# Labbeti/conette-audio-captioning

Hardware: AMD Instinct MI355X
Metric: clips_per_sec (higher is better)
Workload: dtype bf16; 1 GPU; B=64/GPU x 10 s @ 32 kHz clips, ConvNeXt encoder + beam-3 KV-cached decode (min 3 / max 20 tokens, V=5631), synthetic seeded checkpoint; batch_per_gpu=64, global_batch=64, beam_size=3, parallelism=dp1, world_size_observed=1, allreduce_of_ones=1, decode_group=2, decode_streams=2, encode_streams=1, input_batches_rotated=4

## Files before the change

### conette-audio-captioning_amd/build.py

```python
from __future__ import annotations

import json
import os
import shutil
import subprocess
import sys
from concurrent.futures import ThreadPoolExecutor

HERE = os.path.dirname(os.path.abspath(__file__))
CSRC = os.path.join(HERE, "csrc")
LIB = os.path.join(HERE, "libconette_hip.so")
SOURCES = ["api.hip", "frontend.hip", "encoder.hip", "decoder.hip"]
FLAGS = ["--offload-arch=gfx950", "-O3", "-std=c++17", "-fPIC", "-Wno-unused-value"]
if os.environ.get("CN_G2_PROF"):
    FLAGS.append("-DCN_G2_PROF")
for knob in ("FE_NOFILL", "FE_POISON", "FE_NW", "FE_VARIANT"):
    if os.environ.get(knob):
        FLAGS.append(f"-D{knob}" + ("" if os.environ[knob] == "1" and knob != "FE_NW" else "=" + os.environ[knob]))
if os.environ.get("CN_EXTRA_FLAGS"):
    FLAGS += os.environ["CN_EXTRA_FLAGS"].split()
if os.environ.get("CN_DB_ROWS"):
    FLAGS.append("-DDB_ROWS=" + os.environ["CN_DB_ROWS"])
if os.environ.get("CN_DB_ROWS_SP"):
    FLAGS.append("-DDB_ROWS_SP=" + os.environ["CN_DB_ROWS_SP"])
if os.environ.get("CN_DB_WIDE_ROWS"):
    FLAGS.append("-DDB_WIDE_ROWS=" + os.environ["CN_DB_WIDE_ROWS"])
if os.environ.get("CN_DB_WIDE_ROWS_SP"):
    FLAGS.append("-DDB_WIDE_ROWS_SP=" + os.environ["CN_DB_WIDE_ROWS_SP"])
if os.environ.get("CN_DB_WIDE_R"):
    FLAGS.append("-DDB_WIDE_R=" + os.environ["CN_DB_WIDE_R"])
for _k in ("CN_DW96_S", "CN_DW96_TH", "CN_DW192_S", "CN_DW192_TH"):
    if os.environ.get(_k):
        FLAGS.append(f"-D{_k}=" + os.environ[_k])
if os.environ.get("CN_FW_SPLIT"):
    FLAGS.append("-DCN_FW_SPLIT=" + os.environ["CN_FW_SPLIT"])
if os.environ.get("CN_FW_TH"):
    FLAGS.append("-DCN_FW_TH=" + os.environ["CN_FW_TH"])


def hipcc() -> str:
    for cand in (shutil.which("hipcc"), "/opt/rocm/bin/hipcc"):
        if cand and os.path.exists(cand):
            return cand
    raise RuntimeError("hipcc not found")


FILE_FLAGS = {} if os.environ.get("CN_ALLOW_PK_HAZARD") else {"frontend.hip": ["-fno-slp-vectorize"], "decoder.hip": ["-fno-slp-vectorize"]}


SIDECAR = os.path.join(HERE, "libconette_hip.build.json")
# ... 121 lines not shown
```

### conette-audio-captioning_amd/csrc/api.hip

```cpp
#include <math.h>
#include <stdarg.h>
#include <stdlib.h>

#include <string>
#include <unordered_map>
#include <vector>

#include "ctx.h"
#include <algorithm>
#include "mlp_rc2.h"
#include "mlp_rs16.h"
#include "mlp_sp.h"
#include "down_fused.h"

static thread_local char g_err[512] = "";

void cn_set_error(const char* fmt, ...) {
  va_list ap;
  va_start(ap, fmt);
  vsnprintf(g_err, sizeof(g_err), fmt, ap);
  va_end(ap);
}

extern "C" const char* conette_last_error(void) { return g_err; }
// ... 227 lines not shown
  }
  conette_ctx* ctx = new conette_ctx();
  memset(ctx, 0, sizeof(*ctx));
  ctx->cfg = *cfg;
  ctx->rt = new CnRuntime();
  ctx->esize = (cfg->precision == CONETTE_PREC_BF16 || cfg->precision == CONETTE_PREC_F16) ? 2 : 4;
  ctx->f16 = cfg->precision == CONETTE_PREC_F16 ? 1 : 0;
  ctx->sp16 = cfg->precision == CONETTE_PREC_F16X2 ? 1 : 0;
  {
    int dev = 0, n_cu = 0;
    if (hipGetDevice(&dev) != hipSuccess || hipDeviceGetAttribute(&n_cu, hipDeviceAttributeMultiprocessorCount, dev) != hipSuccess ||
        n_cu <= 0)
      n_cu = 256;
    ctx->n_cu = n_cu;
  }
  size_t total = (1 << 20) + (size_t)CN_N_BINS * CN_N_MELS * 4;
  for (int i = 0; i < n_tensors; ++i) total += cn_align((size_t)numel[i] * 4) + 256;
  if (cfg->precision == CONETTE_PREC_F16X2) {
    total += 8u << 20;
    total += (size_t)cfg->n_layers * ((size_t)12 * 131072 + (size_t)(cfg->d_ff / 256 + 1) * 4 * 131072 + 4096);
  }
  ctx->arena_bytes = total;
  hipError_t e = hipMalloc((void**)&ctx->arena, total);
  if (e != hipSuccess) {
    cn_set_error("create: hipMalloc(%zu) -> %s", total, hipGetErrorString(e));
    delete ctx->rt;
    delete ctx;
    return CN_ERR_HIP;
  }
  Builder B;
// ... 424 lines not shown
```

### conette-audio-captioning_amd/csrc/ctx.h

```cpp
#pragma once
#include "../../include/conette_hip.h"
#include "common.h"

#define CN_N_MELS 224
#define CN_N_FFT 1024
#define CN_HOP 320
#define CN_N_BINS 513
#define CN_N_TAGS 527
#define CN_FEAT 768
#define CN_MAX_LAYERS 12

static const int CN_DEPTHS[4] = {3, 3, 9, 3};
static const int CN_DIMS[4] = {96, 192, 384, 768};

struct CnBlockW {
  const float* dw_w;
  const unsigned* dw_wp;
  const float* dw_b;
  const float* ln_w;
  const float* ln_b;
  const void* w1;
  const float* b1;
  const void* w2;
  const float* b2;
// ... 59 lines not shown
  const float* norm_b;
  const void* head_w;
  const float* head_b;
  const void* proj_w;
  const float* proj_b;
  const void* kv_w;
  const float* kv_b;
  CnLayerW layers[CN_MAX_LAYERS];
  const float* emb;
  const float* pe;
  int pe_len;
  const void* cls_w;
  const float* cls_b;
  int n_cu;
  int enc_reserved_cus;
  int forcing_stepwise;
  int score_vsplit;
  char* arena;
  size_t arena_bytes;
  size_t arena_used;
};

void cn_prof_begin(conette_ctx* ctx, int cls, hipStream_t s);
void cn_prof_end(conette_ctx* ctx, int cls, hipStream_t s);
struct CnProfScope {
  conette_ctx* ctx;
  int cls;
  hipStream_t s;
  CnProfScope(conette_ctx* c, int k, hipStream_t st) : ctx(c), cls(k), s(st) {
    if (ctx->prof_mask & (1u << cls)) cn_prof_begin(ctx, cls, s);
// ... 23 lines not shown
```

### conette-audio-captioning_amd/csrc/decoder.hip

```cpp
#include "ctx.h"
#include <stdlib.h>

#include <type_traits>

#include "gemm2.h"
#include "dec_ffn.h"
#include "dec_score.h"

#define CN_MAX_BEAM 16
#define CN_MAX_PRED 64
#define FF2_SPLITS 8
static int ff2_splits_default() { return 4; }

template <typename T>
__global__ void cn_cvt_kernel(const float* __restrict__ in, T* __restrict__ out, size_t n) {
  for (size_t i = (size_t)blockIdx.x * blockDim.x + threadIdx.x; i < n; i += (size_t)gridDim.x * blockDim.x)
    out[i] = cn_from_f32<T>(in[i]);
}

__global__ void cn_init_state_kernel(int B, int beam, int maxp, const int* __restrict__ bos, int* n_active, int* slot,
                                     float* sum_lp, int* prefix, int* anc, int* cur_tok, int* out_preds,
                                     float* out_avg, int* out_len, int* sizes, int pad_id, int* trace_sel,
                                     float* trace_val, int* live, float* margins) {
  const int R = B * beam;
// ... 1180 lines not shown
    if (value < 0) {
      cn_set_error("set_option: score vocabulary split %d < 0", value);
      return CN_ERR_ARG;
    }
    ctx->score_vsplit = value;
    return CN_OK;
  }
  if (option == CONETTE_OPT_ENCODE_RESERVED_CUS) {
    if (value < 0 || value > ctx->n_cu / 2) {
      cn_set_error("set_option: reserved CUs %d outside 0 .. %d", value, ctx->n_cu / 2);
      return CN_ERR_ARG;
    }
    ctx->enc_reserved_cus = value;
    return CN_OK;
  }
  cn_set_error("set_option: unknown option %d", option);
  return CN_ERR_ARG;
}

template <typename... A>
static int dec_check_model(const conette_ctx* ctx, const char* who, int len, int min_pred, const char* len_fmt, A... len_args) {
  if (len < 1 || len > CN_MAX_PRED || len > ctx->pe_len || min_pred < 0) {
    cn_set_error(len_fmt, len_args...);
    return CN_ERR_ARG;
  }
  if (ctx->cfg.d_model != 256 || ctx->cfg.nhead != 8) {
    cn_set_error("%s: kernels are specialised for d_model=256, nhead=8", who);
    return CN_ERR_ARG;
  }
  return CN_OK;
// ... 387 lines not shown
```

### conette-audio-captioning_amd/csrc/down_fused.h

```cpp
#pragma once
__device__ void cn_watch_stat(float v);
#include "mlp_rc2.h"

template <int CP> struct DownGeom {
  static constexpr int K = 4 * CP, N = 2 * CP, KS = K / 16, NT = N / 32, CH = CP / 16;
  static constexpr size_t STREAM_BYTES = (size_t)KS * NT * 1024;
  static constexpr size_t TOTAL_BYTES = STREAM_BYTES + N * 4;
};

template <typename HT>
static __global__ void pk_down_fused(const float* __restrict__ src, const float* __restrict__ g, const float* __restrict__ b,
                                     const float* __restrict__ bias, int N, int C, HT* __restrict__ dst) {
  const int K = 4 * C, KS = K / 16, NT = N / 32;
  const int u = blockIdx.x * blockDim.x + threadIdx.x;
  if (u < N) {
    float a = bias[u];
    for (int k = 0; k < K; ++k) a = fmaf(src[((size_t)u * C + k % C) * 4 + k / C], b[k % C], a);
    ((float*)((char*)dst + (size_t)KS * NT * 1024))[u] = a;
  }
  if (u >= KS * NT * 64) return;
  const int l = u & 63, t = (u >> 6) % NT, s = (u >> 6) / NT;
  const int n = 32 * t + cn_rc2_chan(l & 31);
#pragma unroll
  for (int i = 0; i < 8; ++i) {
// ... 106 lines not shown
    constexpr int s = Q / G::NT, t = Q % G::NT;
    acc[t] = cn_mma32(f[Q % R], a[s], acc[t]);
    __builtin_amdgcn_sched_barrier(0);
    if constexpr (Q + 1 < NM) step<Q + 1>(wl, a, acc, f);
  }
  template <int Q>
  static __device__ __forceinline__ void run(const char* wl, const cn_h8<HT> (&a)[G::KS], f32x16 (&acc)[G::NT]) {
    cn_h8<HT> f[R];
#pragma unroll
    for (int q = 0; q < PRE; ++q) f[q] = *(const cn_h8<HT>*)(wl + q * 1024);
    __builtin_amdgcn_sched_barrier(0);
    step<0>(wl, a, acc, f);
  }
};

template <int CP, int NW, typename HT, typename XT>
__global__ __launch_bounds__(NW * 64) void cn_down_fused_kernel(const XT* __restrict__ X, int H, int W, long P,
                                                                const HT* __restrict__ WS, XT* __restrict__ OUT) {
  typedef DownGeom<CP> G;
  constexpr int KS = G::KS, NT = G::NT, CH = G::CH, N = G::N;
  extern __shared__ __attribute__((aligned(16))) char smem[];
  const int tid = threadIdx.x, lane = tid & 63;
  const int wave = __builtin_amdgcn_readfirstlane(tid >> 6);
  constexpr int PIECES = (int)(G::STREAM_BYTES / 1024);
  for (int i = wave; i < PIECES; i += NW)
    __builtin_amdgcn_global_load_lds((const __attribute__((address_space(1))) void*)((const char*)WS + (size_t)i * 1024 + lane * 16),
                                     (__attribute__((address_space(3))) void*)(smem + i * 1024), 16, 0, 0);
  const float* biasp = (const float*)((const char*)WS + G::STREAM_BYTES);
  const long n_tiles = (P + 31) >> 5;
  const long t_lo = (long)blockIdx.x * n_tiles / gridDim.x, t_hi = (long)(blockIdx.x + 1) * n_tiles / gridDim.x;
  asm volatile("s_waitcnt vmcnt(0)" ::: "memory");
  __syncthreads();
  const char* wl = smem + lane * 16;
  for (long tile = t_lo + wave; tile < t_hi; tile += NW) {
    cn_h8<HT> a[KS];
    cn_down_operand<CP, 0, 4, HT, XT>(X, H, W, P, tile, lane, a);
    f32x16 acc[NT];
#pragma unroll
    for (int t = 0; t < NT; ++t)
#pragma unroll
      for (int i = 0; i < 16; ++i) acc[t][i] = 0.f;
    DownMma<CP, HT>::template run<0>(wl, a, acc);
    cn_down_store<CP, XT>(OUT, biasp, P, tile, lane, acc);
  }
}

template <int CP, int NW, typename HT, typename XT>
static int cn_launch_down_fused(const XT* X, int B, int H, int W, const void* WS, XT* OUT, int n_blocks, hipStream_t s) {
  typedef DownGeom<CP> G;
  constexpr int SMEM = (int)G::STREAM_BYTES;
  static_assert(SMEM <= 160 * 1024, "the packed weights must fit in LDS");
  const long P = (long)B * (H / 2) * (W / 2);
  CN_TRY(cn_configure_lds((const void*)cn_down_fused_kernel<CP, NW, HT, XT>, SMEM));
  const int grid = cn_rc2_grid((int)((P + 31) / 32), NW, n_blocks);
  hipLaunchKernelGGL((cn_down_fused_kernel<CP, NW, HT, XT>), dim3((unsigned)grid), dim3(NW * 64), SMEM, s, X, H, W, P, (const HT*)WS, OUT);
  CN_LAUNCH_CHECK();
  return CN_OK;
}

template <int CP, int NW, int KSTEP, int NST, typename HT> struct DownRing {
  typedef DownGeom<CP> G;
  static constexpr int NT = G::NT, KS = G::KS, NSTEP = KS / KSTEP, FR = KSTEP * NT, SB = FR * 1024;
  static constexpr int DPW = FR / NW, PRE = 6, R = PRE + 1;
  static_assert(KS % KSTEP == 0 && NSTEP % NST == 0 && FR % NW == 0, "ring geometry");
  static constexpr int SMEM = NST * SB;

  static __device__ __forceinline__ void stage(const char* wsrc, char* smem, int wave, int g) {
    const char* src = wsrc + (size_t)(g % NSTEP) * SB;
    char* dst = smem + (g % NST) * SB;
#pragma unroll
// ... 82 lines not shown
```

### conette-audio-captioning_amd/csrc/encoder.hip

```cpp
#include <stddef.h>

#include "ctx.h"
#include <type_traits>

__device__ int g_cn_nonfinite;
__device__ __forceinline__ void cn_watch_stat(float v) {
  if (!(__builtin_fabsf(v) <= 3.0e38f)) atomicAdd(&g_cn_nonfinite, 1);
}

#include "gemm2.h"
#include "mlp_rc2.h"
#include "mlp_rs16.h"
#include "mlp_sp.h"
#include "down_fused.h"

template <typename XT>
__global__ __launch_bounds__(256) void cn_stem_mfma_kernel(const float* __restrict__ in, int F, int H0, long n_pos,
                                                           const float* __restrict__ w , const float* __restrict__ bias,
                                                           const float* __restrict__ ln_w, const float* __restrict__ ln_b,
                                                           XT* __restrict__ out) {
  __shared__ __attribute__((aligned(16))) float s_p[3 * 96];
  for (int i = threadIdx.x; i < 3 * 96; i += 256) s_p[i] = i < 96 ? bias[i] : i < 192 ? ln_w[i - 96] : ln_b[i - 192];
  const int lane = threadIdx.x & 63, j = lane & 31, h = lane >> 5;
  float a[3][8];
#pragma unroll
  for (int t = 0; t < 3; ++t)
#pragma unroll
    for (int s = 0; s < 8; ++s) a[t][s] = w[(4 * (s >> 1) + 2 * h + (s & 1)) * 96 + 32 * t + cn_rc2_chan(j)];
  __syncthreads();
  const long n_tiles = (n_pos + 31) >> 5;
  const long n_waves = (long)gridDim.x * 4;
  for (long tile = (long)blockIdx.x * 4 + (threadIdx.x >> 6); tile < n_tiles; tile += n_waves) {
    const long pos = tile * 32 + j;
    const long p = pos < n_pos ? pos : n_pos - 1;
    const int wq = (int)(p % 56);
// ... 732 lines not shown
    g.W[i] = g.W[i - 1] / 2;
  }
  return g;
}

extern "C" int32_t conette_num_frames(int32_t n_samples) { return n_samples / CN_HOP + 1; }
extern "C" int32_t conette_num_audio_frames(int32_t n_samples) { return enc_geom(n_samples).H[3]; }

struct EncWs {
  float* logmel;
  void* x;
  void* y;
  void* h;
  void* fe_t;
  void* clip_t;
  size_t total;
};
static EncWs enc_ws(const conette_ctx* ctx, int B, int L, char* base) {
  const EncGeom g = enc_geom(L);
  const size_t es = ctx->esize;
  const size_t n0 = (size_t)B * g.H[0] * g.W[0] * 96;
  EncWs w;
  size_t off = 0;
  auto take = [&](size_t bytes) {
    char* p = base ? base + off : nullptr;
    off += cn_align(bytes);
    return p;
  };
  w.logmel = (float*)take((size_t)B * g.F * CN_N_MELS * 4);
  w.x = take((n0 + 32 * 96) * 4);
  w.y = take((n0 + 32 * 96) * es);
  w.h = take(n0 * 4 * es);
  w.fe_t = take((size_t)B * g.H[3] * CN_FEAT * es);
  w.clip_t = take((size_t)B * CN_FEAT * es);
  w.total = off;
  return w;
}

extern "C" size_t conette_encode_workspace_bytes(const conette_ctx* ctx, int32_t batch, int32_t n_samples) {
  return enc_ws(ctx, batch, n_samples, nullptr).total;
}

template <typename T, typename XT>
static int dwconv_dispatch(int C, const XT* x, int B, int H, int W, const CnBlockW& bw, T* y, hipStream_t s) {
  switch (C) {
    case 96: return launch_dwconv<T, XT, 96, CN_DW96_S, sizeof(XT) == 2 ? CN_DW96_TH : 8>(x, B, H, W, bw, y, s);
    case 192: return launch_dwconv<T, XT, 192, CN_DW192_S, sizeof(XT) == 2 ? CN_DW192_TH : 8>(x, B, H, W, bw, y, s);
    case 384:
      if (W == 14) return launch_dwconv_fw<T, XT, 384, 14, CN_FW_TH, CN_FW_SPLIT>(x, B, H, bw, y, s);
// ... 17 lines not shown
  if (dst) {
    hipLaunchKernelGGL(cn_tap_widen_kernel, dim3((unsigned)((n + 255) / 256 < 4096 ? (n + 255) / 256 : 4096)), dim3(256), 0, s, src, dst, n);
    CN_LAUNCH_CHECK();
  }
  return CN_OK;
}

template <typename T, typename XT>
static int encode_impl(conette_ctx* ctx, const float* wave, int B, int L, float* frame_embs, float* clip_probs,
                       const conette_encode_taps* taps, char* wsp, hipStream_t s) {
  const EncGeom g = enc_geom(L);
  EncWs ws = enc_ws(ctx, B, L, wsp);
  T* y = (T*)ws.y;
  T* hbuf = (T*)ws.h;
  XT* const wsx = (XT*)ws.x;
  {
    CnProfScope ps(ctx, CONETTE_PROF_FRONTEND, s);
    CN_TRY(cn_frontend(ctx, wave, B, L, ws.logmel, s));
  }
  if (taps) CN_TRY(tap_copy(taps->logmel, ws.logmel, (size_t)B * g.F * CN_N_MELS, s));
  {
    const long n_pos = (long)B * g.H[0] * g.W[0];
    CnProfScope ps(ctx, CONETTE_PROF_STEM, s);
    const long n_tiles = (n_pos + 31) / 32;
    const unsigned grid = (unsigned)std::min<long>((n_tiles + 3) / 4, 8L * ctx->n_cu);
    hipLaunchKernelGGL((cn_stem_mfma_kernel<XT>), dim3(grid), dim3(256), 0, s, ws.logmel, g.F, g.H[0], n_pos, ctx->stem_w, ctx->stem_b,
                       ctx->stem_ln_w, ctx->stem_ln_b, wsx);
    CN_LAUNCH_CHECK();
    if (taps) CN_TRY(tap_copy(taps->stem, wsx, (size_t)n_pos * 96, s));
  }
  XT* xc = wsx;
  int blk = 0;
  for (int st = 0; st < 4; ++st) {
    const int C = CN_DIMS[st], H = g.H[st], W = g.W[st];
    const long P = (long)B * H * W;
    if (st > 0) {
      const int Cp = CN_DIMS[st - 1], Hp = g.H[st - 1], Wp = g.W[st - 1];
      const long n_in = (long)B * Hp * Wp;
      const CnDownW& dw = ctx->down[st - 1];
      CnProfScope ps(ctx, CONETTE_PROF_DOWNSAMPLE, s);
      bool fused_down = false;
      if constexpr (CnIsH16<T>::value) if (Cp <= 192 && dw.fused != nullptr) {
        XT* xo = xc == wsx ? (XT*)ws.h : wsx;
        const int nb = ctx->n_cu - ctx->enc_reserved_cus;
        if (Cp == 96) CN_TRY((cn_launch_down_fused<96, 8, T, XT>(xc, B, Hp, Wp, dw.fused, xo, nb, s)));
        else CN_TRY((cn_launch_down_fused_ring<192, 4, 4, 3, T, XT>(xc, B, Hp, Wp, dw.fused, xo, nb, s)));
        xc = xo;
        if (taps) CN_TRY(tap_copy(taps->down[st], xc, (size_t)P * C, s));
        fused_down = true;
      }
      if (!fused_down) {
      const int ppb = Cp == 96 ? 32 : 16;
      const dim3 pg((unsigned)((n_in + ppb - 1) / ppb));
      if (Cp == 96)
        hipLaunchKernelGGL((cn_ln_patchify_kernel<T, XT, 96>), pg, dim3(256), 0, s, xc, Hp, Wp, n_in, dw.ln_w, dw.ln_b, y);
      else if (Cp == 192)
        hipLaunchKernelGGL((cn_ln_patchify_kernel<T, XT, 192>), pg, dim3(256), 0, s, xc, Hp, Wp, n_in, dw.ln_w, dw.ln_b, y);
      else
        hipLaunchKernelGGL((cn_ln_patchify_kernel<T, XT, 384>), pg, dim3(256), 0, s, xc, Hp, Wp, n_in, dw.ln_w, dw.ln_b, y);
      CN_LAUNCH_CHECK();
// ... 1 lines not shown
      CN_TRY(cn_mm(y, 4 * Cp, (const T*)dw.w, 4 * Cp, (int)P, C, 4 * Cp, epi, s));
      xc = wsx;
      if (taps) CN_TRY(tap_copy(taps->down[st], xc, (size_t)P * C, s));
      }
    }
    for (int b = 0; b < CN_DEPTHS[st]; ++b, ++blk) {
      const CnBlockW& bw = ctx->blocks[blk];
      {
        CnProfScope ps(ctx, CONETTE_PROF_DWCONV_LN, s);
        CN_TRY((dwconv_dispatch<T, XT>(C, xc, B, H, W, bw, y, s)));
      }
      bool fused = false;
      if constexpr (std::is_same<T, sp16_t>::value) {
        if (bw.mlp_sp != nullptr && C <= 192) {
          CnProfScope ps(ctx, CONETTE_PROF_PW1_GEMM, s);
          const int nb = ctx->n_cu - ctx->enc_reserved_cus;
          if (C == 96) CN_TRY((cn_launch_mlp_sp_ring<96, CN_SP_NW96, CN_SP_NST96>(y, bw.mlp_sp, xc, (int)P, nb, s)));
          else CN_TRY((cn_launch_mlp_sp_ring<192, 8, 3>(y, bw.mlp_sp, xc, (int)P, nb, s)));
          fused = true;
        }
      }
      if constexpr (CnIsH16<T>::value) if (!fused) {
        if (bw.mlp_stream != nullptr && C <= 384) {
          CnProfScope ps(ctx, CONETTE_PROF_PW1_GEMM, s);
          const T* wsm = (const T*)bw.mlp_stream;
          if (C == 96) CN_TRY((cn_launch_mlp_rc2_resident<96, 12, 1>(y, wsm, xc, (int)P, ctx->n_cu - ctx->enc_reserved_cus, s)));
          else if (C == 192) CN_TRY((cn_launch_mlp_rc2_ring<192, 8, CN_RC2_NCK(192), CN_RC2_NCK(192) == 2 ? 3 : 5>(y, wsm, xc, (int)P, ctx->n_cu - ctx->enc_reserved_cus, s)));
          else CN_TRY((cn_launch_mlp_rs16<384, 4, 3, 8>(y, wsm, xc, (int)P, ctx->n_cu - ctx->enc_reserved_cus, s)));
          fused = true;
        }
      }
      if (!fused) {
        {
          CnProfScope ps(ctx, CONETTE_PROF_PW1_GEMM, s);
          constexpr int kAct = CnGeluAct<T>::value;
          EpiBiasAct<T, kAct> e1{bw.b1, hbuf, 4 * C, kAct};
          CN_TRY(cn_mm(y, C, (const T*)bw.w1, C, (int)P, 4 * C, C, e1, s));
        }
        {
          CnProfScope ps(ctx, CONETTE_PROF_PW2_GEMM, s);
          EpiResidT<XT> e2{bw.b2, bw.scale, xc, xc, C};
          CN_TRY(cn_mm(hbuf, 4 * C, (const T*)bw.w2, 4 * C, (int)P, C, 4 * C, e2, s));
        }
// ... 92 lines not shown
```

### conette-audio-captioning_amd/csrc/mlp_rc2.h

```cpp
#pragma once
#include "common.h"

template <int C, int NCK> struct Rc2Geom {
  static constexpr int KS1 = C / 16, NT2 = C / 32, NCH = C / 8;
  static constexpr int F1 = KS1 + 1, F2 = 2 * NT2;
  static constexpr int NSTEP = NCH / NCK;
  static constexpr int FRAGS = NCK * (F1 + F2);
  static constexpr int STEP_BYTES = FRAGS * 1024;
  static constexpr size_t STREAM_BYTES = (size_t)NSTEP * STEP_BYTES;
  static constexpr size_t TOTAL_BYTES = STREAM_BYTES + NT2 * 1024;
};
__host__ __device__ constexpr int cn_rc2_chan(int m) { return (m & 19) | ((m & 4) << 1) | ((m & 8) >> 1); }

#define CN_MLP_XSCALE 0.5f
template <typename HT> __device__ __forceinline__ float cn_gelu_mlp(float x) {
  return cn_gelu_e1_half<__is_same(HT, half_t) ? 5 : 3>(x);
}

template <typename HT>
static __global__ void pk_mlp_rc2(const float* __restrict__ W1, const float* __restrict__ b1, const float* __restrict__ W2,
                           const float* __restrict__ b2, const float* __restrict__ scale, int C, int NCK,
                           HT* __restrict__ dst) {
  const int KS1 = C / 16, NT2 = C / 32, NCH = C / 8, F1 = KS1 + 1, F2 = 2 * NT2, FRAGS = NCK * (F1 + F2), NSTEP = NCH / NCK;
  const int u = blockIdx.x * blockDim.x + threadIdx.x;
// ... 201 lines not shown
      if ((r & 3) + 8 * (r >> 2) < plim) {
#pragma unroll
        for (int t = 0; t < NT2; ++t) row[voff + 32 * t] = O[t][r] + bb[t];
      }
    }
  }
};

static inline int cn_rc2_grid(int n_tiles, int waves_per_block, int max_blocks) {
  const int block_tiles = cn_cdiv(n_tiles, waves_per_block);
  if (max_blocks < 1) max_blocks = 1;
  const int rounds = cn_cdiv(block_tiles, max_blocks);
  return cn_cdiv(block_tiles, rounds);
}

template <int C, int NW, int NCK, typename HT = bf16_t, int ABL = 0, typename XT = float>
__global__ __launch_bounds__(NW * 64) void cn_mlp_rc2_resident_kernel(const HT* __restrict__ Y, const HT* __restrict__ WS,
                                                                      XT* __restrict__ X, int M) {
  typedef Rc2Geom<C, NCK> G;
  typedef Rc2Wave<C, NCK, HT, XT> W;
  typedef cn_h8<HT> hx8;
  extern __shared__ __attribute__((aligned(16))) char smem[];
  const int tid = threadIdx.x, lane = tid & 63;
  const int wave = __builtin_amdgcn_readfirstlane(tid >> 6);
  constexpr int TOTAL = G::NSTEP * G::FRAGS;
  for (int i = wave; i < TOTAL; i += NW)
    __builtin_amdgcn_global_load_lds((const __attribute__((address_space(1))) void*)((const char*)WS + (size_t)i * 1024 + lane * 16),
                                     (__attribute__((address_space(3))) void*)(smem + i * 1024), 16, 0, 0);
  const char* bbf = (const char*)WS + G::STREAM_BYTES + lane * 16;
  const int n_tiles = (M + 31) >> 5;
  const int t_lo = (int)((long)blockIdx.x * n_tiles / gridDim.x), t_hi = (int)((long)(blockIdx.x + 1) * n_tiles / gridDim.x);
  hx8 ones;
#pragma unroll
  for (int i = 0; i < 8; ++i) ones[i] = (HT)((lane < 32 && i < 2) ? 1.0f : 0.0f);
  hx8 fy[G::KS1];
  int tile = t_lo + wave;
  if (tile < t_hi) W::load_y(Y, tile * 32, lane, fy);
  asm volatile("s_waitcnt vmcnt(0)" ::: "memory");
  __syncthreads();
  const char* wl = smem + lane * 16;
  for (; tile < t_hi; tile += NW) {
    f32x16 O[G::NT2];
    if constexpr (ABL & 1) {
#pragma unroll
      for (int t = 0; t < G::NT2; ++t) O[t] = W::zero16();
    } else {
      W::init_o(X, bbf, ones, tile * 32, lane, O);
    }
#pragma unroll 1
    for (int j = 0; j < G::NSTEP; ++j) W::step(wl + j * G::STEP_BYTES, fy, ones, O);
    if constexpr (!(ABL & 8))
      if (tile + NW < t_hi) W::load_y(Y, (tile + NW) * 32, lane, fy);
    if constexpr (ABL & 2) {
      if (O[0][0] == 12345.678f) W::store_o(X, tile * 32, M, lane, O);
    } else {
      W::store_o(X, tile * 32, M, lane, O);
    }
  }
}

template <int C, int NW, int NCK, int ABL = 0, typename HT, typename XT>
static int cn_launch_mlp_rc2_resident(const HT* Y, const HT* WS, XT* X, int M, int n_blocks, hipStream_t s) {
  constexpr int SMEM = (int)Rc2Geom<C, NCK>::STREAM_BYTES;
  static_assert(SMEM <= 160 * 1024, "resident variant: the weight stream must fit in LDS");
  CN_TRY(cn_configure_lds((const void*)cn_mlp_rc2_resident_kernel<C, NW, NCK, HT, ABL, XT>, SMEM));
  const int grid = cn_rc2_grid((M + 31) / 32, NW, n_blocks);
  hipLaunchKernelGGL((cn_mlp_rc2_resident_kernel<C, NW, NCK, HT, ABL, XT>), dim3((unsigned)grid), dim3(NW * 64), SMEM, s, Y, WS, X, M);
  CN_LAUNCH_CHECK();
  return CN_OK;
}

template <int C, int NW, int NCK, int NST, int PROF = 0, typename HT = bf16_t, typename XT = float>
__global__ __launch_bounds__(NW * 64) void cn_mlp_rc2_ring_kernel(const HT* __restrict__ Y, const HT* __restrict__ WS,
                                                                  XT* __restrict__ X, int M, unsigned long long* prof = nullptr) {
  unsigned long long tacc[5] = {0, 0, 0, 0, 0}, tprev = 0, nstep = 0;
  auto stamp = [&](int i) {
    if constexpr (PROF) {
      const unsigned long long t = clock64();
      tacc[i] += t - tprev;
      tprev = t;
    }
  };
  if constexpr (PROF) tprev = clock64();
  typedef Rc2Geom<C, NCK> G;
  typedef Rc2Wave<C, NCK, HT, XT> W;
  typedef cn_h8<HT> hx8;
  constexpr int FR = G::FRAGS, SB = G::STEP_BYTES;
  constexpr int DPW_LO = FR / NW, N_HI = FR % NW;
  extern __shared__ __attribute__((aligned(16))) char smem[];
  const int tid = threadIdx.x, lane = tid & 63;
  const int wave = __builtin_amdgcn_readfirstlane(tid >> 6);
  const char* bbf = (const char*)WS + G::STREAM_BYTES + lane * 16;

  const int n_tiles = (M + 31) >> 5;
  const int t_lo = (int)((long)blockIdx.x * n_tiles / gridDim.x), t_hi = (int)((long)(blockIdx.x + 1) * n_tiles / gridDim.x);
  const int max_it = (t_hi - t_lo + NW - 1) / NW;

  const unsigned voff = lane * 16;
  const unsigned lds0 = cn_lds_addr(smem);
  auto stage = [&](int g) {
    const char* src = (const char*)WS + (size_t)(g % G::NSTEP) * SB;
    const unsigned dst = lds0 + (unsigned)((g % NST) * SB);
#pragma unroll
    for (int i = 0; i < DPW_LO + 1; ++i) {
      const int piece = wave + i * NW;
      if (i < DPW_LO || wave < N_HI) cn_dma16_s(src + piece * 1024, voff, dst + piece * 1024);
    }
  };
  hx8 ones;
#pragma unroll
  for (int i = 0; i < 8; ++i) ones[i] = (HT)((lane < 32 && i < 2) ? 1.0f : 0.0f);

#pragma unroll
  for (int g = 0; g < NST - 1; ++g) stage(g);
  hx8 fy[G::KS1];
  if (t_lo + wave < t_hi) W::load_y(Y, (t_lo + wave) * 32, lane, fy);
  const char* wl = smem + lane * 16;
  int g = 0;
  for (int it = 0; it < max_it; ++it) {
    const int tile = t_lo + wave + it * NW;
    const bool valid = tile < t_hi;
    f32x16 O[G::NT2];
    if (valid) W::init_o(X, bbf, ones, tile * 32, lane, O);
    {
      __builtin_amdgcn_s_waitcnt(0x0F70);
    }
    for (int j = 0; j < G::NSTEP; ++j, ++g) {
      stamp(4);
      if (N_HI > 0 && wave < N_HI) asm volatile("s_waitcnt vmcnt(%0)" ::"n"((NST - 2) * (DPW_LO + 1)) : "memory");
      else asm volatile("s_waitcnt vmcnt(%0)" ::"n"((NST - 2) * DPW_LO) : "memory");
      stamp(0);
      __builtin_amdgcn_s_barrier();
      stamp(1);
      stage(g + NST - 1);
      stamp(2);
      if (valid) W::step(wl + (g % NST) * SB, fy, ones, O);
      stamp(3);
      if constexpr (PROF) nstep += valid;
    }
    if (tile + NW < t_hi) W::load_y(Y, (tile + NW) * 32, lane, fy);
    if (valid) W::store_o(X, tile * 32, M, lane, O);
  }
  asm volatile("s_waitcnt vmcnt(0)" ::: "memory");
  if constexpr (PROF) {
    if (lane == 0 && prof) {
#pragma unroll
      for (int i = 0; i < 5; ++i) atomicAdd(prof + i, tacc[i]);
      atomicAdd(prof + 5, nstep);
    }
  }
}

template <int C, int NW, int NCK, int NST, int PROF = 0, typename HT, typename XT>
static int cn_launch_mlp_rc2_ring(const HT* Y, const HT* WS, XT* X, int M, int n_blocks, hipStream_t s,
                                  unsigned long long* prof = nullptr) {
  constexpr int SMEM = NST * Rc2Geom<C, NCK>::STEP_BYTES;
  static_assert(SMEM <= 160 * 1024, "ring must fit in LDS");
  CN_TRY(cn_configure_lds((const void*)cn_mlp_rc2_ring_kernel<C, NW, NCK, NST, PROF, HT, XT>, SMEM));
  const int grid = cn_rc2_grid((M + 31) / 32, NW, n_blocks);
  hipLaunchKernelGGL((cn_mlp_rc2_ring_kernel<C, NW, NCK, NST, PROF, HT, XT>), dim3((unsigned)grid), dim3(NW * 64), SMEM, s, Y, WS, X, M, prof);
  CN_LAUNCH_CHECK();
  return CN_OK;
}
```

### conette-audio-captioning_amd/engine.py

```python
from __future__ import annotations

import ctypes as C
import os
from typing import Any, Dict, Optional, Tuple

import torch

_HERE = os.path.dirname(os.path.abspath(__file__))
LIB_PATH = os.path.join(_HERE, "libconette_hip.so")

PREC_F32 = 0
PREC_BF16 = 1
PREC_F16X2 = 2
PREC_F16 = 4
N_MELS = 224
FEAT = 768
N_TAGS = 527

EXPORTS = (
    "conette_last_error", "conette_abi_version", "conette_create", "conette_destroy", "conette_num_frames",
    "conette_num_audio_frames", "conette_encode_workspace_bytes", "conette_decode_workspace_bytes",
    "conette_frontend_logmel", "conette_encode", "conette_decode", "conette_resample", "conette_resample_len",
    "conette_set_option", "conette_profile_enable", "conette_profile_read", "conette_stream_create_masked",
    "conette_stream_destroy", "conette_forcing_workspace_bytes", "conette_forcing",
# ... 4 lines not shown
    "mixed16": {"greedy": (0.032, 0.0, 0.0), "beam": (0.045, 0.0, 0.005), "wide": (0.08, 0.0, 0.005)},
    "f16": {"greedy": (0.063, 0.0, 0.0), "beam": (0.082, 0.0, 0.008), "wide": (0.13, 0.0, 0.008)},
    "bf16+f16dec": {"greedy": (0.20, 0.0, 0.0), "beam": (0.37, 0.0, 0.026), "wide": (0.65, 0.0, 0.05)},
    "bf16": {"greedy": (0.39, 0.0, 0.0), "beam": (0.58, 0.0, 0.05), "wide": (1.0, 0.0, 0.08)},
}


def cert_kind(beam: int) -> str:
    return "greedy" if int(beam) == 1 else ("beam" if int(beam) <= 5 else "wide")


CERT_DEFAULT_BASE = "mixed16"
OPT_DECODE_GRAPH = 1
OPT_DECODE_FUSION = 2
OPT_ENCODE_RESERVED_CUS = 3
OPT_FORCING_STEPWISE = 4
OPT_SCORE_VSPLIT = 5
MAX_DECODE_GRAPHS = 64
PROF_CLASSES = ("frontend", "stem", "dwconv_ln", "pw1_gemm", "pw2_gemm", "downsample", "heads", "dec_prepare",
                "dec_gemm", "dec_attn", "dec_misc", "search")


class ConetteConfigC(C.Structure):
    _fields_ = [(n, C.c_int32) for n in ("precision", "vocab_size", "d_model", "nhead", "n_layers", "d_ff", "pad_id",
                                         "bos_id", "eos_id")] + [("reserved", C.c_int32 * 7)]


class EncodeTapsC(C.Structure):
    _fields_ = [("struct_bytes", C.c_size_t), ("logmel", C.c_void_p), ("stem", C.c_void_p), ("stage_block0", C.c_void_p * 4),
                ("stage", C.c_void_p * 4), ("down", C.c_void_p * 4), ("block", C.c_void_p * 18)]
# ... 539 lines not shown
                            exact: bool = False) -> torch.Tensor:
        return self._decode_buffers(b, t, int(beam), int(max_pred), False, False, slot, margins, exact)["fe"]

    def set_decode_graph(self, enabled: bool) -> None:
        _check(self.lib.conette_set_option(self._ctx_dec, OPT_DECODE_GRAPH, int(bool(enabled))), "set_option")

    def set_decode_fusion(self, enabled: bool) -> None:
        _check(self.lib.conette_set_option(self._ctx_dec, OPT_DECODE_FUSION, int(bool(enabled))), "set_option")

    def set_forcing_stepwise(self, enabled: bool) -> None:
        _check(self.lib.conette_set_option(self._ctx_dec, OPT_FORCING_STEPWISE, int(bool(enabled))), "set_option")

    def set_encode_reserved_cus(self, n: int) -> None:
        _check(self.lib.conette_set_option(self._ctx, OPT_ENCODE_RESERVED_CUS, int(n)), "set_option")

    def decode_graph_nodes(self) -> int:
        return int(self.lib.conette_decode_graph_nodes(self._ctx_dec))

    _DEC_CLASSES = ("dec_prepare", "dec_gemm", "dec_attn", "dec_misc", "search")

    def profile_enable(self, classes=()) -> None:
        mask_enc = mask_dec = 0
        for c in classes:
            bit = 1 << PROF_CLASSES.index(c)
            if c in self._DEC_CLASSES:
                mask_dec |= bit
            else:
                mask_enc |= bit
        if self._ctx_dec is self._ctx:
            _check(self.lib.conette_profile_enable(self._ctx, mask_enc | mask_dec), "profile_enable")
# ... 24 lines not shown
```

### include/conette_hip.h

```cpp
#ifndef CONETTE_HIP_H
#define CONETTE_HIP_H

#include <stddef.h>
#include <stdint.h>

#ifdef __cplusplus
extern "C" {
#endif

#define CONETTE_ABI_VERSION 3

#define CONETTE_PREC_F32 0
#define CONETTE_PREC_BF16 1
#define CONETTE_PREC_F16X2 2


#define CONETTE_PREC_F16 4

typedef struct conette_ctx conette_ctx;

typedef struct conette_config {
  int32_t precision;
  int32_t vocab_size;
  int32_t d_model;
// ... 72 lines not shown
                   float* sum_lprobs, int32_t* lens, int32_t* out_sizes, float* tok_lprobs, float* step_logits,
                   void* workspace, size_t workspace_bytes, void* stream);

int conette_resample(const float* in, int32_t rows, int32_t n_in, int32_t orig_sr, int32_t new_sr, float* out,
                     void* stream);
int32_t conette_resample_len(int32_t n_in, int32_t orig_sr, int32_t new_sr);

int conette_stream_create_masked(const uint32_t* mask_words, int32_t n_words, void** out_stream);
int conette_stream_destroy(void* stream);

#define CONETTE_OPT_DECODE_GRAPH 1
#define CONETTE_OPT_DECODE_FUSION 2
#define CONETTE_OPT_ENCODE_RESERVED_CUS 3
#define CONETTE_OPT_FORCING_STEPWISE 4
#define CONETTE_OPT_SCORE_VSPLIT 5
int conette_set_option(conette_ctx* ctx, int32_t option, int32_t value);

int32_t conette_decode_graph_nodes(const conette_ctx* ctx);
#define CONETTE_MAX_DECODE_GRAPHS 64

#define CONETTE_PROF_FRONTEND 0
#define CONETTE_PROF_STEM 1
#define CONETTE_PROF_DWCONV_LN 2
#define CONETTE_PROF_PW1_GEMM 3
#define CONETTE_PROF_PW2_GEMM 4
#define CONETTE_PROF_DOWNSAMPLE 5
#define CONETTE_PROF_HEADS 6
#define CONETTE_PROF_DEC_PREPARE 7
#define CONETTE_PROF_DEC_GEMM 8
#define CONETTE_PROF_DEC_ATTN 9
// ... 11 lines not shown
```

Measured before the change: 13370 clips/s.

## Add atomic work-claiming tile scheduler for encoder MLP and downsample kernels

Adds a dynamic tile-claiming mode to the ConvNeXt encoder's rc2 MLP kernels and fused downsample kernel. Each wave pulls its next tile from a global atomic counter instead of a static contiguous range, which is meant to even out load imbalance and tail effects when encoder kernels share CUs with concurrent decode streams. The counters are zeroed by the stem kernel, and per-wave slots are spaced to avoid contention. The default enables it for the 96-channel MLP and downsample only. It adds atomic traffic and one readfirstlane per tile, and the ring variant gains extra LDS for the shared draw queue.

```diff
diff --git a/conette-audio-captioning_amd/build.py b/conette-audio-captioning_amd/build.py
--- a/conette-audio-captioning_amd/build.py
+++ b/conette-audio-captioning_amd/build.py
@@ -34,6 +34,8 @@
         FLAGS.append(f"-D{_k}=" + os.environ[_k])
 if os.environ.get("CN_FW_SPLIT"):
     FLAGS.append("-DCN_FW_SPLIT=" + os.environ["CN_FW_SPLIT"])
+if os.environ.get("CN_ENC_CLAIM"):
+    FLAGS.append("-DCONETTE_CLAIM_DEFAULT=" + os.environ["CN_ENC_CLAIM"])
 if os.environ.get("CN_FW_TH"):
     FLAGS.append("-DCN_FW_TH=" + os.environ["CN_FW_TH"])
 
diff --git a/conette-audio-captioning_amd/csrc/api.hip b/conette-audio-captioning_amd/csrc/api.hip
--- a/conette-audio-captioning_amd/csrc/api.hip
+++ b/conette-audio-captioning_amd/csrc/api.hip
@@ -265,6 +265,7 @@
       n_cu = 256;
     ctx->n_cu = n_cu;
   }
+  ctx->enc_claim = CONETTE_CLAIM_DEFAULT;
   size_t total = (1 << 20) + (size_t)CN_N_BINS * CN_N_MELS * 4;
   for (int i = 0; i < n_tensors; ++i) total += cn_align((size_t)numel[i] * 4) + 256;
   if (cfg->precision == CONETTE_PREC_F16X2) {
diff --git a/conette-audio-captioning_amd/csrc/ctx.h b/conette-audio-captioning_amd/csrc/ctx.h
--- a/conette-audio-captioning_amd/csrc/ctx.h
+++ b/conette-audio-captioning_amd/csrc/ctx.h
@@ -97,6 +97,8 @@
   const float* cls_b;
   int n_cu;
   int enc_reserved_cus;
+  int enc_max_blocks;
+  int enc_claim;
   int forcing_stepwise;
   int score_vsplit;
   char* arena;
diff --git a/conette-audio-captioning_amd/csrc/decoder.hip b/conette-audio-captioning_amd/csrc/decoder.hip
--- a/conette-audio-captioning_amd/csrc/decoder.hip
+++ b/conette-audio-captioning_amd/csrc/decoder.hip
@@ -1218,6 +1218,22 @@
     ctx->enc_reserved_cus = value;
     return CN_OK;
   }
+  if (option == CONETTE_OPT_ENCODE_MAX_BLOCKS) {
+    if (value < 0) {
+      cn_set_error("set_option: encode block cap %d < 0", value);
+      return CN_ERR_ARG;
+    }
+    ctx->enc_max_blocks = value;
+    return CN_OK;
+  }
+  if (option == CONETTE_OPT_ENCODE_CLAIM) {
+    if (value < -1 || (value >= 0 && (value & ~CONETTE_CLAIM_ALL))) {
+      cn_set_error("set_option: encode claim mask %d has bits outside %d", value, CONETTE_CLAIM_ALL);
+      return CN_ERR_ARG;
+    }
+    ctx->enc_claim = value < 0 ? CONETTE_CLAIM_DEFAULT : value;
+    return CN_OK;
+  }
   cn_set_error("set_option: unknown option %d", option);
   return CN_ERR_ARG;
 }
diff --git a/conette-audio-captioning_amd/csrc/down_fused.h b/conette-audio-captioning_amd/csrc/down_fused.h
--- a/conette-audio-captioning_amd/csrc/down_fused.h
+++ b/conette-audio-captioning_amd/csrc/down_fused.h
@@ -144,9 +144,10 @@
   }
 };
 
-template <int CP, int NW, typename HT, typename XT>
+template <int CP, int NW, typename HT, typename XT, bool DYN = false>
 __global__ __launch_bounds__(NW * 64) void cn_down_fused_kernel(const XT* __restrict__ X, int H, int W, long P,
-                                                                const HT* __restrict__ WS, XT* __restrict__ OUT) {
+                                                                const HT* __restrict__ WS, XT* __restrict__ OUT,
+                                                                unsigned* site = nullptr) {
   typedef DownGeom<CP> G;
   constexpr int KS = G::KS, NT = G::NT, CH = G::CH, N = G::N;
   extern __shared__ __attribute__((aligned(16))) char smem[];
@@ -158,11 +159,21 @@
                                      (__attribute__((address_space(3))) void*)(smem + i * 1024), 16, 0, 0);
   const float* biasp = (const float*)((const char*)WS + G::STREAM_BYTES);
   const long n_tiles = (P + 31) >> 5;
-  const long t_lo = (long)blockIdx.x * n_tiles / gridDim.x, t_hi = (long)(blockIdx.x + 1) * n_tiles / gridDim.x;
+  long tile, t_hi;
+  unsigned* word = nullptr;
+  if constexpr (DYN) {
+    static_assert(NW <= CN_CLAIM_SITE_WORDS / CN_CLAIM_SLOT_WORDS, "one slot per wave");
+    word = site + wave * CN_CLAIM_SLOT_WORDS;
+    tile = (long)blockIdx.x * NW + wave, t_hi = n_tiles;
+  } else {
+    tile = (long)blockIdx.x * n_tiles / gridDim.x + wave, t_hi = (long)(blockIdx.x + 1) * n_tiles / gridDim.x;
+  }
   asm volatile("s_waitcnt vmcnt(0)" ::: "memory");
   __syncthreads();
   const char* wl = smem + lane * 16;
-  for (long tile = t_lo + wave; tile < t_hi; tile += NW) {
+  while (tile < t_hi) {
+    int drawn = 0;
+    if constexpr (DYN) drawn = cn_claim_issue(word, lane);
     cn_h8<HT> a[KS];
     cn_down_operand<CP, 0, 4, HT, XT>(X, H, W, P, tile, lane, a);
     f32x16 acc[NT];
@@ -172,18 +183,30 @@
       for (int i = 0; i < 16; ++i) acc[t][i] = 0.f;
     DownMma<CP, HT>::template run<0>(wl, a, acc);
     cn_down_store<CP, XT>(OUT, biasp, P, tile, lane, acc);
+    if constexpr (DYN) tile = (long)cn_claim_value(drawn) * NW + wave;
+    else tile += NW;
   }
 }
 
 template <int CP, int NW, typename HT, typename XT>
-static int cn_launch_down_fused(const XT* X, int B, int H, int W, const void* WS, XT* OUT, int n_blocks, hipStream_t s) {
+static int cn_launch_down_fused(const XT* X, int B, int H, int W, const void* WS, XT* OUT, int n_blocks, hipStream_t s,
+                                unsigned* claim_site = nullptr) {
   typedef DownGeom<CP> G;
   constexpr int SMEM = (int)G::STREAM_BYTES;
   static_assert(SMEM <= 160 * 1024, "the packed weights must fit in LDS");
   const long P = (long)B * (H / 2) * (W / 2);
+  if (claim_site) {
+    CN_TRY(cn_configure_lds((const void*)cn_down_fused_kernel<CP, NW, HT, XT, true>, SMEM));
+    const int grid = cn_claim_grid((int)((P + 31) / 32), NW, n_blocks);
+    hipLaunchKernelGGL((cn_down_fused_kernel<CP, NW, HT, XT, true>), dim3((unsigned)grid), dim3(NW * 64), SMEM, s, X, H, W, P, (const HT*)WS, OUT,
+                       claim_site);
+    CN_LAUNCH_CHECK();
+    return CN_OK;
+  }
   CN_TRY(cn_configure_lds((const void*)cn_down_fused_kernel<CP, NW, HT, XT>, SMEM));
   const int grid = cn_rc2_grid((int)((P + 31) / 32), NW, n_blocks);
-  hipLaunchKernelGGL((cn_down_fused_kernel<CP, NW, HT, XT>), dim3((unsigned)grid), dim3(NW * 64), SMEM, s, X, H, W, P, (const HT*)WS, OUT);
+  hipLaunchKernelGGL((cn_down_fused_kernel<CP, NW, HT, XT>), dim3((unsigned)grid), dim3(NW * 64), SMEM, s, X, H, W, P, (const HT*)WS, OUT,
+                     (unsigned*)nullptr);
   CN_LAUNCH_CHECK();
   return CN_OK;
 }
diff --git a/conette-audio-captioning_amd/csrc/encoder.hip b/conette-audio-captioning_amd/csrc/encoder.hip
--- a/conette-audio-captioning_amd/csrc/encoder.hip
+++ b/conette-audio-captioning_amd/csrc/encoder.hip
@@ -14,11 +14,15 @@
 #include "mlp_sp.h"
 #include "down_fused.h"
 
+#define CN_ENC_CLAIM_SITES 17
+
 template <typename XT>
 __global__ __launch_bounds__(256) void cn_stem_mfma_kernel(const float* __restrict__ in, int F, int H0, long n_pos,
                                                            const float* __restrict__ w , const float* __restrict__ bias,
                                                            const float* __restrict__ ln_w, const float* __restrict__ ln_b,
-                                                           XT* __restrict__ out) {
+                                                           XT* __restrict__ out, unsigned* __restrict__ claim, int n_claim_slots) {
+  if (claim && blockIdx.x == 0)
+    for (int i = threadIdx.x; i < n_claim_slots; i += 256) claim[i * CN_CLAIM_SLOT_WORDS] = 0u;
   __shared__ __attribute__((aligned(16))) float s_p[3 * 96];
   for (int i = threadIdx.x; i < 3 * 96; i += 256) s_p[i] = i < 96 ? bias[i] : i < 192 ? ln_w[i - 96] : ln_b[i - 192];
   const int lane = threadIdx.x & 63, j = lane & 31, h = lane >> 5;
@@ -781,6 +785,7 @@
   void* h;
   void* fe_t;
   void* clip_t;
+  unsigned* claim;
   size_t total;
 };
 static EncWs enc_ws(const conette_ctx* ctx, int B, int L, char* base) {
@@ -800,6 +805,7 @@
   w.h = take(n0 * 4 * es);
   w.fe_t = take((size_t)B * g.H[3] * CN_FEAT * es);
   w.clip_t = take((size_t)B * CN_FEAT * es);
+  w.claim = (unsigned*)take((size_t)CN_ENC_CLAIM_SITES * CN_CLAIM_SITE_WORDS * sizeof(unsigned));
   w.total = off;
   return w;
 }
@@ -847,6 +853,10 @@
   T* y = (T*)ws.y;
   T* hbuf = (T*)ws.h;
   XT* const wsx = (XT*)ws.x;
+  int nb = ctx->n_cu - ctx->enc_reserved_cus;
+  if (ctx->enc_max_blocks > 0) nb = std::min(nb, ctx->enc_max_blocks);
+  const int claim = CnIsH16<T>::value ? ctx->enc_claim : 0;
+  auto site = [&](int bit, int i) { return (claim & bit) ? ws.claim + (size_t)i * CN_CLAIM_SITE_WORDS : (unsigned*)nullptr; };
   {
     CnProfScope ps(ctx, CONETTE_PROF_FRONTEND, s);
     CN_TRY(cn_frontend(ctx, wave, B, L, ws.logmel, s));
@@ -858,7 +868,8 @@
     const long n_tiles = (n_pos + 31) / 32;
     const unsigned grid = (unsigned)std::min<long>((n_tiles + 3) / 4, 8L * ctx->n_cu);
     hipLaunchKernelGGL((cn_stem_mfma_kernel<XT>), dim3(grid), dim3(256), 0, s, ws.logmel, g.F, g.H[0], n_pos, ctx->stem_w, ctx->stem_b,
-                       ctx->stem_ln_w, ctx->stem_ln_b, wsx);
+                       ctx->stem_ln_w, ctx->stem_ln_b, wsx, claim ? ws.claim : (unsigned*)nullptr,
+                       CN_ENC_CLAIM_SITES * (CN_CLAIM_SITE_WORDS / CN_CLAIM_SLOT_WORDS));
     CN_LAUNCH_CHECK();
     if (taps) CN_TRY(tap_copy(taps->stem, wsx, (size_t)n_pos * 96, s));
   }
@@ -875,8 +886,7 @@
       bool fused_down = false;
       if constexpr (CnIsH16<T>::value) if (Cp <= 192 && dw.fused != nullptr) {
         XT* xo = xc == wsx ? (XT*)ws.h : wsx;
-        const int nb = ctx->n_cu - ctx->enc_reserved_cus;
-        if (Cp == 96) CN_TRY((cn_launch_down_fused<96, 8, T, XT>(xc, B, Hp, Wp, dw.fused, xo, nb, s)));
+        if (Cp == 96) CN_TRY((cn_launch_down_fused<96, 8, T, XT>(xc, B, Hp, Wp, dw.fused, xo, nb, s, site(CONETTE_CLAIM_DOWN96, 15))));
         else CN_TRY((cn_launch_down_fused_ring<192, 4, 4, 3, T, XT>(xc, B, Hp, Wp, dw.fused, xo, nb, s)));
         xc = xo;
         if (taps) CN_TRY(tap_copy(taps->down[st], xc, (size_t)P * C, s));
@@ -908,7 +918,6 @@
       if constexpr (std::is_same<T, sp16_t>::value) {
         if (bw.mlp_sp != nullptr && C <= 192) {
           CnProfScope ps(ctx, CONETTE_PROF_PW1_GEMM, s);
-          const int nb = ctx->n_cu - ctx->enc_reserved_cus;
           if (C == 96) CN_TRY((cn_launch_mlp_sp_ring<96, CN_SP_NW96, CN_SP_NST96>(y, bw.mlp_sp, xc, (int)P, nb, s)));
           else CN_TRY((cn_launch_mlp_sp_ring<192, 8, 3>(y, bw.mlp_sp, xc, (int)P, nb, s)));
           fused = true;
@@ -918,9 +927,9 @@
         if (bw.mlp_stream != nullptr && C <= 384) {
           CnProfScope ps(ctx, CONETTE_PROF_PW1_GEMM, s);
           const T* wsm = (const T*)bw.mlp_stream;
-          if (C == 96) CN_TRY((cn_launch_mlp_rc2_resident<96, 12, 1>(y, wsm, xc, (int)P, ctx->n_cu - ctx->enc_reserved_cus, s)));
-          else if (C == 192) CN_TRY((cn_launch_mlp_rc2_ring<192, 8, CN_RC2_NCK(192), CN_RC2_NCK(192) == 2 ? 3 : 5>(y, wsm, xc, (int)P, ctx->n_cu - ctx->enc_reserved_cus, s)));
-          else CN_TRY((cn_launch_mlp_rs16<384, 4, 3, 8>(y, wsm, xc, (int)P, ctx->n_cu - ctx->enc_reserved_cus, s)));
+          if (C == 96) CN_TRY((cn_launch_mlp_rc2_resident<96, 12, 1>(y, wsm, xc, (int)P, nb, s, site(CONETTE_CLAIM_MLP96, blk))));
+          else if (C == 192) CN_TRY((cn_launch_mlp_rc2_ring<192, 8, CN_RC2_NCK(192), CN_RC2_NCK(192) == 2 ? 3 : 5>(y, wsm, xc, (int)P, nb, s, nullptr, site(CONETTE_CLAIM_MLP192, blk))));
+          else CN_TRY((cn_launch_mlp_rs16<384, 4, 3, 8>(y, wsm, xc, (int)P, nb, s)));
           fused = true;
         }
       }
diff --git a/conette-audio-captioning_amd/csrc/mlp_rc2.h b/conette-audio-captioning_amd/csrc/mlp_rc2.h
--- a/conette-audio-captioning_amd/csrc/mlp_rc2.h
+++ b/conette-audio-captioning_amd/csrc/mlp_rc2.h
@@ -239,9 +239,23 @@
   return cn_cdiv(block_tiles, rounds);
 }
 
-template <int C, int NW, int NCK, typename HT = bf16_t, int ABL = 0, typename XT = float>
+#define CN_CLAIM_SLOT_WORDS 32
+#define CN_CLAIM_SITE_WORDS 512
+static __device__ __forceinline__ int cn_claim_issue(unsigned* word, int lane) {
+  int v = 0;
+  if (lane == 0) v = (int)atomicAdd(word, 1u);
+  return v;
+}
+static __device__ __forceinline__ int cn_claim_value(int v) {
+  return (int)gridDim.x + __builtin_amdgcn_readfirstlane(v);
+}
+static inline int cn_claim_grid(int n_tiles, int waves_per_block, int max_blocks) {
+  return std::max(1, std::min(cn_cdiv(n_tiles, waves_per_block), max_blocks));
+}
+
+template <int C, int NW, int NCK, typename HT = bf16_t, int ABL = 0, typename XT = float, bool DYN = false>
 __global__ __launch_bounds__(NW * 64) void cn_mlp_rc2_resident_kernel(const HT* __restrict__ Y, const HT* __restrict__ WS,
-                                                                      XT* __restrict__ X, int M) {
+                                                                      XT* __restrict__ X, int M, unsigned* site = nullptr) {
   typedef Rc2Geom<C, NCK> G;
   typedef Rc2Wave<C, NCK, HT, XT> W;
   typedef cn_h8<HT> hx8;
@@ -254,17 +268,27 @@
                                      (__attribute__((address_space(3))) void*)(smem + i * 1024), 16, 0, 0);
   const char* bbf = (const char*)WS + G::STREAM_BYTES + lane * 16;
   const int n_tiles = (M + 31) >> 5;
-  const int t_lo = (int)((long)blockIdx.x * n_tiles / gridDim.x), t_hi = (int)((long)(blockIdx.x + 1) * n_tiles / gridDim.x);
+  int tile, t_hi;
+  unsigned* word = nullptr;
+  if constexpr (DYN) {
+    static_assert(NW <= CN_CLAIM_SITE_WORDS / CN_CLAIM_SLOT_WORDS, "one slot per wave");
+    word = site + wave * CN_CLAIM_SLOT_WORDS;
+    tile = (int)blockIdx.x * NW + wave, t_hi = n_tiles;
+  } else {
+    const int t_lo = (int)((long)blockIdx.x * n_tiles / gridDim.x);
+    tile = t_lo + wave, t_hi = (int)((long)(blockIdx.x + 1) * n_tiles / gridDim.x);
+  }
   hx8 ones;
 #pragma unroll
   for (int i = 0; i < 8; ++i) ones[i] = (HT)((lane < 32 && i < 2) ? 1.0f : 0.0f);
   hx8 fy[G::KS1];
-  int tile = t_lo + wave;
   if (tile < t_hi) W::load_y(Y, tile * 32, lane, fy);
   asm volatile("s_waitcnt vmcnt(0)" ::: "memory");
   __syncthreads();
   const char* wl = smem + lane * 16;
-  for (; tile < t_hi; tile += NW) {
+  while (tile < t_hi) {
+    int drawn = 0;
+    if constexpr (DYN) drawn = cn_claim_issue(word, lane);
     f32x16 O[G::NT2];
     if constexpr (ABL & 1) {
 #pragma unroll
@@ -274,30 +298,44 @@
     }
 #pragma unroll 1
     for (int j = 0; j < G::NSTEP; ++j) W::step(wl + j * G::STEP_BYTES, fy, ones, O);
+    int next = tile + NW;
+    if constexpr (DYN) next = cn_claim_value(drawn) * NW + wave;
     if constexpr (!(ABL & 8))
-      if (tile + NW < t_hi) W::load_y(Y, (tile + NW) * 32, lane, fy);
+      if (next < t_hi) W::load_y(Y, next * 32, lane, fy);
     if constexpr (ABL & 2) {
       if (O[0][0] == 12345.678f) W::store_o(X, tile * 32, M, lane, O);
     } else {
       W::store_o(X, tile * 32, M, lane, O);
     }
+    tile = next;
   }
 }
 
 template <int C, int NW, int NCK, int ABL = 0, typename HT, typename XT>
-static int cn_launch_mlp_rc2_resident(const HT* Y, const HT* WS, XT* X, int M, int n_blocks, hipStream_t s) {
+static int cn_launch_mlp_rc2_resident(const HT* Y, const HT* WS, XT* X, int M, int n_blocks, hipStream_t s,
+                                      unsigned* claim_site = nullptr) {
   constexpr int SMEM = (int)Rc2Geom<C, NCK>::STREAM_BYTES;
   static_assert(SMEM <= 160 * 1024, "resident variant: the weight stream must fit in LDS");
+  if (claim_site) {
+    CN_TRY(cn_configure_lds((const void*)cn_mlp_rc2_resident_kernel<C, NW, NCK, HT, ABL, XT, true>, SMEM));
+    const int grid = cn_claim_grid((M + 31) / 32, NW, n_blocks);
+    hipLaunchKernelGGL((cn_mlp_rc2_resident_kernel<C, NW, NCK, HT, ABL, XT, true>), dim3((unsigned)grid), dim3(NW * 64), SMEM, s, Y, WS, X, M,
+                       claim_site);
+    CN_LAUNCH_CHECK();
+    return CN_OK;
+  }
   CN_TRY(cn_configure_lds((const void*)cn_mlp_rc2_resident_kernel<C, NW, NCK, HT, ABL, XT>, SMEM));
   const int grid = cn_rc2_grid((M + 31) / 32, NW, n_blocks);
-  hipLaunchKernelGGL((cn_mlp_rc2_resident_kernel<C, NW, NCK, HT, ABL, XT>), dim3((unsigned)grid), dim3(NW * 64), SMEM, s, Y, WS, X, M);
+  hipLaunchKernelGGL((cn_mlp_rc2_resident_kernel<C, NW, NCK, HT, ABL, XT>), dim3((unsigned)grid), dim3(NW * 64), SMEM, s, Y, WS, X, M,
+                     (unsigned*)nullptr);
   CN_LAUNCH_CHECK();
   return CN_OK;
 }
 
-template <int C, int NW, int NCK, int NST, int PROF = 0, typename HT = bf16_t, typename XT = float>
+template <int C, int NW, int NCK, int NST, int PROF = 0, typename HT = bf16_t, typename XT = float, bool DYN = false>
 __global__ __launch_bounds__(NW * 64) void cn_mlp_rc2_ring_kernel(const HT* __restrict__ Y, const HT* __restrict__ WS,
-                                                                  XT* __restrict__ X, int M, unsigned long long* prof = nullptr) {
+                                                                  XT* __restrict__ X, int M, unsigned long long* prof = nullptr,
+                                                                  unsigned* site = nullptr) {
   unsigned long long tacc[5] = {0, 0, 0, 0, 0}, tprev = 0, nstep = 0;
   auto stamp = [&](int i) {
     if constexpr (PROF) {
@@ -318,8 +356,11 @@
   const char* bbf = (const char*)WS + G::STREAM_BYTES + lane * 16;
 
   const int n_tiles = (M + 31) >> 5;
-  const int t_lo = (int)((long)blockIdx.x * n_tiles / gridDim.x), t_hi = (int)((long)(blockIdx.x + 1) * n_tiles / gridDim.x);
+  const int t_lo = DYN ? 0 : (int)((long)blockIdx.x * n_tiles / gridDim.x);
+  const int t_hi = DYN ? n_tiles : (int)((long)(blockIdx.x + 1) * n_tiles / gridDim.x);
   const int max_it = (t_hi - t_lo + NW - 1) / NW;
+  static_assert(!DYN || G::NSTEP >= 2, "the draw is published one step before the tile's last");
+  volatile int* q = (volatile int*)(smem + NST * SB);
 
   const unsigned voff = lane * 16;
   const unsigned lds0 = cn_lds_addr(smem);
@@ -339,11 +380,13 @@
 #pragma unroll
   for (int g = 0; g < NST - 1; ++g) stage(g);
   hx8 fy[G::KS1];
-  if (t_lo + wave < t_hi) W::load_y(Y, (t_lo + wave) * 32, lane, fy);
+  int unit = 0, par = 0, drawn = 0;
+  if constexpr (DYN) unit = (int)blockIdx.x;
+  if (t_lo + unit * NW + wave < t_hi) W::load_y(Y, (t_lo + unit * NW + wave) * 32, lane, fy);
   const char* wl = smem + lane * 16;
   int g = 0;
-  for (int it = 0; it < max_it; ++it) {
-    const int tile = t_lo + wave + it * NW;
+  for (int it = 0; DYN ? unit < max_it : it < max_it; ++it) {
+    const int tile = t_lo + wave + (DYN ? unit : it) * NW;
     const bool valid = tile < t_hi;
     f32x16 O[G::NT2];
     if (valid) W::init_o(X, bbf, ones, tile * 32, lane, O);
@@ -359,11 +402,24 @@
       stamp(1);
       stage(g + NST - 1);
       stamp(2);
+      if constexpr (DYN)
+        if (j == 0 && wave == 0) drawn = cn_claim_issue(site, lane);
       if (valid) W::step(wl + (g % NST) * SB, fy, ones, O);
       stamp(3);
       if constexpr (PROF) nstep += valid;
-    }
-    if (tile + NW < t_hi) W::load_y(Y, (tile + NW) * 32, lane, fy);
+      if constexpr (DYN)
+        if (j == G::NSTEP - 2 && wave == 0) {
+          q[par ^ 1] = cn_claim_value(drawn);
+          asm volatile("s_waitcnt lgkmcnt(0)" ::: "memory");
+        }
+    }
+    int next = tile + NW;
+    if constexpr (DYN) {
+      par ^= 1;
+      unit = __builtin_amdgcn_readfirstlane(q[par]);
+      next = unit * NW + wave;
+    }
+    if (next < t_hi) W::load_y(Y, next * 32, lane, fy);
     if (valid) W::store_o(X, tile * 32, M, lane, O);
   }
   asm volatile("s_waitcnt vmcnt(0)" ::: "memory");
@@ -378,12 +434,21 @@
 
 template <int C, int NW, int NCK, int NST, int PROF = 0, typename HT, typename XT>
 static int cn_launch_mlp_rc2_ring(const HT* Y, const HT* WS, XT* X, int M, int n_blocks, hipStream_t s,
-                                  unsigned long long* prof = nullptr) {
-  constexpr int SMEM = NST * Rc2Geom<C, NCK>::STEP_BYTES;
+                                  unsigned long long* prof = nullptr, unsigned* claim_site = nullptr) {
+  constexpr int SMEM = NST * Rc2Geom<C, NCK>::STEP_BYTES + 16;
   static_assert(SMEM <= 160 * 1024, "ring must fit in LDS");
+  if (claim_site) {
+    CN_TRY(cn_configure_lds((const void*)cn_mlp_rc2_ring_kernel<C, NW, NCK, NST, PROF, HT, XT, true>, SMEM));
+    const int grid = cn_claim_grid((M + 31) / 32, NW, n_blocks);
+    hipLaunchKernelGGL((cn_mlp_rc2_ring_kernel<C, NW, NCK, NST, PROF, HT, XT, true>), dim3((unsigned)grid), dim3(NW * 64), SMEM, s, Y, WS, X, M,
+                       prof, claim_site);
+    CN_LAUNCH_CHECK();
+    return CN_OK;
+  }
   CN_TRY(cn_configure_lds((const void*)cn_mlp_rc2_ring_kernel<C, NW, NCK, NST, PROF, HT, XT>, SMEM));
   const int grid = cn_rc2_grid((M + 31) / 32, NW, n_blocks);
-  hipLaunchKernelGGL((cn_mlp_rc2_ring_kernel<C, NW, NCK, NST, PROF, HT, XT>), dim3((unsigned)grid), dim3(NW * 64), SMEM, s, Y, WS, X, M, prof);
+  hipLaunchKernelGGL((cn_mlp_rc2_ring_kernel<C, NW, NCK, NST, PROF, HT, XT>), dim3((unsigned)grid), dim3(NW * 64), SMEM, s, Y, WS, X, M, prof,
+                     (unsigned*)nullptr);
   CN_LAUNCH_CHECK();
   return CN_OK;
 }
diff --git a/conette-audio-captioning_amd/engine.py b/conette-audio-captioning_amd/engine.py
--- a/conette-audio-captioning_amd/engine.py
+++ b/conette-audio-captioning_amd/engine.py
@@ -42,6 +42,9 @@
 OPT_DECODE_GRAPH = 1
 OPT_DECODE_FUSION = 2
 OPT_ENCODE_RESERVED_CUS = 3
+OPT_ENCODE_MAX_BLOCKS = 6
+OPT_ENCODE_CLAIM = 7
+CLAIM_MLP96, CLAIM_MLP192, CLAIM_DOWN96, CLAIM_ALL = 1, 2, 8, 11
 OPT_FORCING_STEPWISE = 4
 OPT_SCORE_VSPLIT = 5
 MAX_DECODE_GRAPHS = 64
@@ -611,6 +614,12 @@
     def set_encode_reserved_cus(self, n: int) -> None:
         _check(self.lib.conette_set_option(self._ctx, OPT_ENCODE_RESERVED_CUS, int(n)), "set_option")
 
+    def set_encode_max_blocks(self, n: int) -> None:
+        _check(self.lib.conette_set_option(self._ctx, OPT_ENCODE_MAX_BLOCKS, int(n)), "set_option")
+
+    def set_encode_claim(self, mask: Optional[int]) -> None:
+        _check(self.lib.conette_set_option(self._ctx, OPT_ENCODE_CLAIM, -1 if mask is None else int(mask)), "set_option")
+
     def decode_graph_nodes(self) -> int:
         return int(self.lib.conette_decode_graph_nodes(self._ctx_dec))
 
diff --git a/include/conette_hip.h b/include/conette_hip.h
--- a/include/conette_hip.h
+++ b/include/conette_hip.h
@@ -110,6 +110,15 @@
 #define CONETTE_OPT_ENCODE_RESERVED_CUS 3
 #define CONETTE_OPT_FORCING_STEPWISE 4
 #define CONETTE_OPT_SCORE_VSPLIT 5
+#define CONETTE_OPT_ENCODE_MAX_BLOCKS 6
+#define CONETTE_OPT_ENCODE_CLAIM 7
+#define CONETTE_CLAIM_MLP96 1
+#define CONETTE_CLAIM_MLP192 2
+#define CONETTE_CLAIM_DOWN96 8
+#define CONETTE_CLAIM_ALL 11
+#ifndef CONETTE_CLAIM_DEFAULT
+#define CONETTE_CLAIM_DEFAULT (CONETTE_CLAIM_MLP96 | CONETTE_CLAIM_DOWN96)
+#endif
 int conette_set_option(conette_ctx* ctx, int32_t option, int32_t value);
 
 int32_t conette_decode_graph_nodes(const conette_ctx* ctx);
```

Measured after the change: 13370 clips/s (median of 2 runs). About the same (+0.0%).
